# LiWentomng/OrientedRepPoints

Measured on NVIDIA H100. Metric: 1024x1024 tiles/sec, higher is better.
Workload: dtype f16x3

## Files before the change

### orientedreppoints_b200/csrc/common.cuh

```cuda
#pragma once
#include <cuda_runtime.h>
#include <stdint.h>
#include <stdio.h>
#include <string.h>

#include "../../include/orp_b200.h"

namespace orp {

extern thread_local char g_err[512];
extern int64_t g_launches;
extern int g_timing;

inline int fail(int code, const char *fmt, const char *a = "", const char *b = "")
{
    snprintf(g_err, sizeof(g_err), fmt, a, b);
    return code;
}

#define ORP_CUDA(expr)                                                                          \
    do {                                                                                        \
        cudaError_t e__ = (expr);                                                               \
        if (e__ != cudaSuccess) return ::orp::fail(ORP_ECUDA, "%s: %s", #expr, cudaGetErrorString(e__)); \
    } while (0)

#define ORP_LAUNCHED()                                                                          \
    do {                                                                                        \
        __atomic_add_fetch(&::orp::g_launches, 1, __ATOMIC_RELAXED);                            \
        cudaError_t e__ = cudaGetLastError();                                                   \
        if (e__ != cudaSuccess) return ::orp::fail(ORP_ECUDA, "kernel launch: %s", cudaGetErrorString(e__)); \
    } while (0)

inline void count_launches(int n) { __atomic_add_fetch(&g_launches, n, __ATOMIC_RELAXED); }

int ensure_device();

struct Scratch {
    cudaStream_t st;
    void *ptrs[48];
    int n = 0;
    explicit Scratch(cudaStream_t s) : st(s) {}
    ~Scratch() { for (int i = 0; i < n; ++i) cudaFreeAsync(ptrs[i], st); }
    template <typename T> T *get(size_t count)
    {
        void *p = nullptr;
        size_t bytes = (count ? count : 1) * sizeof(T);
        if (n >= 48 || cudaMallocAsync(&p, bytes, st) != cudaSuccess) return nullptr;
        ptrs[n++] = p;
        return static_cast<T *>(p);
    }
};

int run_nms(const float *dets, const int32_t *segments, int n, double thr, int iou_mode, int union_mode,
            int order, int64_t *keep_out, int32_t *num_out, cudaStream_t st, uint8_t *flags_out, bool no_sync,
            int seg_limit ,
            int32_t *overflow_out );

static inline int ceil_div(long long a, long long b) { return (int)((a + b - 1) / b); }

inline int key_bits(uint64_t v)
{
    int b = 1;
    while (b < 64 && (v >> b)) ++b;
    return b;
}

__device__ __forceinline__ uint32_t orderable(float f)
{
    uint32_t u = __float_as_uint(f);
    return (u & 0x80000000u) ? ~u : (u | 0x80000000u);
}

int device_sms(int &sms);

constexpr int kNumSMs = 132;

inline int grid_for(size_t items, int threads)
{
    const size_t g = (items + threads - 1) / threads;
    const size_t cap = kNumSMs * 16;
    return (int)(g < cap ? (g ? g : 1) : cap);
}

}
```

### orientedreppoints_b200/csrc/head_post.cu

```cuda
#include <cub/cub.cuh>

#include "common.cuh"
#include "minrect.cuh"

namespace orp {
namespace {

constexpr int kMaxLevels = 8;
constexpr int kMaxEntries = 80;

struct Levels {
    const float *cls[kMaxEntries], *ref[kMaxEntries];
    int H[kMaxEntries], W[kMaxEntries], stride[kMaxEntries];
    int slot0[kMaxEntries];
    int sort0[kMaxEntries];
    int nent, per_view, B, C, S;
};
static_assert(sizeof(Levels) <= 4000, "the level table is a kernel argument");

__device__ __forceinline__ float sigmoidf_ref(float x) { return 1.0f / (1.0f + expf(-x)); }

__global__ void __launch_bounds__(256)
maxscore_kernel(const __grid_constant__ Levels L, int lev, uint64_t *__restrict__ keys, int32_t *__restrict__ vals)
{
// ... 226 lines not shown
    O.dets = Sc.get<float>(total * 9);
    O.segs = Sc.get<int32_t>(total);
    O.valid = Sc.get<uint8_t>(total);
    O.rp = aug ? nullptr : Sc.get<float>((size_t)B * S * 18);
    O.box = Sc.get<float>((size_t)B * S * 8);
    uint8_t *keep = Sc.get<uint8_t>(total);
    int32_t *counts = Sc.get<int32_t>(B);
    uint64_t *sk1 = Sc.get<uint64_t>(total), *sk2 = Sc.get<uint64_t>(total);
    int32_t *sv1 = Sc.get<int32_t>(total), *sv2 = Sc.get<int32_t>(total);
    size_t tb1 = 0, tb2 = 0;
    if (nsort) cub::DeviceRadixSort::SortPairs(nullptr, tb1, k1, k2, v1, v2, (int)nsort, 0, 64, st);
    const int sel_bits = 32 + key_bits((uint64_t)B - 1);
    cub::DeviceRadixSort::SortPairs(nullptr, tb2, sk1, sk2, sv1, sv2, (int)total, 0, sel_bits, st);
    uint8_t *tmp = Sc.get<uint8_t>(tb1 > tb2 ? tb1 : tb2);
    if (!tmp || !sv2 || !keep) return fail(ORP_ECUDA, "%s: scratch allocation failed", who);

    if (nsort) {
        for (int l = 0; l < L.nent; ++l)
            if (L.sort0[l] >= 0) {
                maxscore_kernel<<<grid_for((size_t)B * H[l] * W[l], 256), 256, 0, st>>>(L, l, k1, v1);
                ORP_LAUNCHED();
            }
        ORP_CUDA(cub::DeviceRadixSort::SortPairs(tmp, tb1, k1, k2, v1, v2, (int)nsort, 0, 64, st));
        count_launches(9);
    }
    const int dgrid = (int)ceil_div((long long)B * S, 128);
    if (aug) decode_kernel<true><<<dgrid, 128, 0, st>>>(L, v2, score_thr, nullptr, view_meta, O);
    else decode_kernel<false><<<dgrid, 128, 0, st>>>(L, v2, score_thr, scale_factor, nullptr, O);
    ORP_LAUNCHED();
    int32_t *nms_ovf = Sc.get<int32_t>(1);
    if (!nms_ovf) return fail(ORP_ECUDA, "%s: scratch allocation failed", who);
    ORP_CUDA(cudaMemsetAsync(nms_ovf, 0, sizeof(int32_t), st));
    rc = run_nms(O.dets, O.segs, (int)total, iou_thr, ORP_NMS_EXACT64, ORP_UNION_NAN_KEEPS, ORP_ORDER_INDEX_ASC, nullptr,
                 nullptr, st, keep, true, B * num_cls, nms_ovf);
    if (rc) return rc;
    ORP_CUDA(cudaMemsetAsync(counts, 0, sizeof(int32_t) * B, st));
    count_kernel<<<dim3(32, B), 256, 0, st>>>(keep, O.valid, (int)per_img, B, counts);
    ORP_LAUNCHED();
    select_keys_kernel<<<grid_for(total, 256), 256, 0, st>>>(keep, O.valid, O.dets, counts, (int)per_img, B, max_per_img, sk1, sv1);
    ORP_LAUNCHED();
    ORP_CUDA(cub::DeviceRadixSort::SortPairs(tmp, tb2, sk1, sk2, sv1, sv2, (int)total, 0, sel_bits, st));
    count_launches((sel_bits + 7) / 8 + 1);
    gather_kernel<<<dim3(ceil_div(max_per_img, 128), B), 128, 0, st>>>(sv2, counts, O.dets, O.rp, O.box, out_scale, (int)per_img,
                                                                     (int)S, num_cls, max_per_img, B, dets_out, labels_out,
                                                                     counts_out, nms_ovf);
    ORP_LAUNCHED();
    return ORP_OK;
}

}
}

extern "C" int orp_head_postprocess(int nlevels, const float *const *cls, const float *const *ref, const int *H,
                                    const int *W, const int *stride, int B, int num_cls, int nms_pre, float score_thr,
                                    double iou_thr, int max_per_img, const float *scale_factor, float *dets_out,
                                    int64_t *labels_out, int32_t *counts_out, void *stream)
{
    return head_post("orp_head_postprocess", 1, nlevels, cls, ref, H, W, stride, B, num_cls, nms_pre, score_thr, iou_thr,
                     max_per_img, scale_factor, nullptr, nullptr, dets_out, labels_out, counts_out, stream);
}

extern "C" int orp_head_postprocess_aug(int nviews, int nlevels, const float *const *cls, const float *const *ref,
                                        const int *H, const int *W, const int *stride, int B, int num_cls, int nms_pre,
                                        float score_thr, double iou_thr, int max_per_img, const float *view_meta,
                                        const float *out_scale, float *dets_out, int64_t *labels_out, int32_t *counts_out,
                                        void *stream)
{
// ... 40 lines not shown
```

### orientedreppoints_b200/csrc/nms.cu

```cuda
#include <cooperative_groups.h>
#include <cub/cub.cuh>
#include <vector>

#include "common.cuh"
#include "geom.cuh"

namespace cg = cooperative_groups;

namespace orp {

struct NmsCounters {
    unsigned long long pairs_swept, pairs_aabb, pairs_clipped, pairs_fp64, edges, suppressing;
    int overflow;
    int rounds;
};

static thread_local int g_last_n;
static thread_local cudaEvent_t g_ev[2] = {nullptr, nullptr};
static thread_local NmsCounters *g_stats_pinned = nullptr;
static thread_local orp_rnms_plan g_last_plan;
static thread_local bool g_have_plan = false;

constexpr float kZeroArea = -2.0f;

__global__ void __launch_bounds__(256)
nms_prep_kernel(const float *__restrict__ dets, int n, uint32_t *__restrict__ score_key, int32_t *__restrict__ iota)
{
    int i = blockIdx.x * blockDim.x + threadIdx.x;
    if (i >= n) return;
    const float *d = dets + (size_t)i * 9;
    const float sc = (__float_as_uint(d[8]) << 1) == 0u ? 0.0f : d[8];
    score_key[i] = ~orderable(sc);
    iota[i] = i;
}

__global__ void __launch_bounds__(256)
nms_rank_kernel(const int32_t *__restrict__ order, int n, int32_t *__restrict__ rank)
{
    int r = blockIdx.x * blockDim.x + threadIdx.x;
    if (r < n) rank[order[r]] = r;
}

struct NmsGlobal {
    unsigned int ymin_key;
    unsigned int maxh_bits;
    unsigned int maxabs_bits;
    double sumh;
    unsigned int count;
};

__device__ __forceinline__ float from_orderable(uint32_t k)
{
    return __uint_as_float((k & 0x80000000u) ? (k & 0x7FFFFFFFu) : ~k);
}

__global__ void __launch_bounds__(256)
nms_boxes_kernel(const float *__restrict__ dets, int n, float4 *__restrict__ baabb, float4 *__restrict__ v01,
                 float4 *__restrict__ v23, float *__restrict__ area, NmsGlobal *__restrict__ G)
{
    __shared__ unsigned int s_ymin, s_maxh, s_cnt, s_maxabs;
    __shared__ float s_sum;
    if (threadIdx.x == 0) { s_ymin = 0xFFFFFFFFu; s_maxh = 0u; s_cnt = 0u; s_sum = 0.f; s_maxabs = 0u; }
    __syncthreads();
    const int i = blockIdx.x * blockDim.x + threadIdx.x;
    if (i < n) {
        const float *d = dets + (size_t)i * 9;
        float c[8];
        bool finite = true;
#pragma unroll
        for (int k = 0; k < 8; ++k) { c[k] = d[k]; finite = finite && isfinite(c[k]); }
        const float xmin = fminf(fminf(c[0], c[2]), fminf(c[4], c[6])), xmax = fmaxf(fmaxf(c[0], c[2]), fmaxf(c[4], c[6]));
        const float ymin = fminf(fminf(c[1], c[3]), fminf(c[5], c[7])), ymax = fmaxf(fmaxf(c[1], c[3]), fmaxf(c[5], c[7]));
        baabb[i] = make_float4(xmin, ymin, xmax, ymax);
        v01[i] = make_float4(c[0], c[1], c[2], c[3]);
        v23[i] = make_float4(c[4], c[5], c[6], c[7]);
        const float ux = c[2] - c[0], uy = c[3] - c[1], vx = c[4] - c[0], vy = c[5] - c[1], wx = c[6] - c[0], wy = c[7] - c[1];
        area[i] = quad_is_convex(c) ? 0.5f * fabsf((ux * vy - uy * vx) + (vx * wy - vy * wx)) : -1.0f;
        if (finite) {
            Pt<double> P[5];
#pragma unroll
            for (int k = 0; k < 4; ++k) { P[k].x = (double)c[2 * k]; P[k].y = (double)c[2 * k + 1]; }
            if (ring_area(P, 4) == 0.0) area[i] = kZeroArea;
        }
        if (finite) {
            atomicMin(&s_ymin, orderable(ymin));
            atomicMax(&s_maxh, __float_as_uint(ymax - ymin));
            atomicMax(&s_maxabs, __float_as_uint(fmaxf(fmaxf(fabsf(xmin), fabsf(xmax)), fmaxf(fabsf(ymin), fabsf(ymax)))));
            atomicAdd(&s_sum, ymax - ymin);
            atomicAdd(&s_cnt, 1u);
        }
    }
    __syncthreads();
    if (threadIdx.x == 0 && s_cnt) {
        atomicMin(&G->ymin_key, s_ymin);
        atomicMax(&G->maxh_bits, s_maxh);
        atomicMax(&G->maxabs_bits, s_maxabs);
        atomicAdd(&G->sumh, (double)s_sum);
        atomicAdd(&G->count, s_cnt);
    }
}

struct Strips {
    float y0, s;
    __device__ __forceinline__ int of(float y) const { return (int)floorf((y - y0) / s); }
};
__device__ __forceinline__ Strips make_strips(const NmsGlobal *G, int R)
{
    Strips S;
    S.y0 = from_orderable(G->ymin_key);
    if (R == 1 || G->count == 0) { S.s = 3.0e38f; return S; }
    const float maxh = __uint_as_float(G->maxh_bits), meanh = (float)(G->sumh / (double)G->count);
    S.s = fmaxf(fmaxf(1.5f * meanh, maxh * (1.0001f / 3.0f)), 1e-6f);
    return S;
}

__global__ void __launch_bounds__(256)
nms_regs_kernel(const float4 *__restrict__ baabb, const int32_t *__restrict__ segments, int n, int R,
                const NmsGlobal *__restrict__ G, uint64_t *__restrict__ keys, int32_t *__restrict__ vals)
{
    const int i = blockIdx.x * blockDim.x + threadIdx.x;
    if (i >= n) return;
    const float4 b = baabb[i];
    const bool finite = isfinite(b.x) && isfinite(b.y) && isfinite(b.z) && isfinite(b.w);
    const Strips S = make_strips(G, R);
    int t0 = 0, t1 = -1;
    if (finite) { t0 = S.of(b.y); t1 = S.of(b.w); if (R == 1) t1 = t0 = 0; if (t1 - t0 > R - 1) t1 = t0 + R - 1; }
    if (R == 1) {
        const uint64_t seg = segments ? (uint64_t)((uint32_t)segments[i] & 0x7FFFFFFFu) : 0ull;
        keys[i] = finite ? ((seg << 32) | orderable(b.x)) : ~0ull;
        vals[i] = i;
        return;
    }
    const uint64_t seg = segments ? (uint64_t)((uint32_t)segments[i] & 0x7FFFu) : 0ull;
    for (int k = 0; k < R; ++k) {
        const int t = t0 + k;
        keys[(size_t)i * R + k] = (t <= t1) ? ((seg << 48) | ((uint64_t)(uint32_t)(t & 0xFFFF) << 32) | orderable(b.x)) : ~0ull;
        vals[(size_t)i * R + k] = i;
    }
}

__global__ void __launch_bounds__(256)
nms_slots_kernel(const uint64_t *__restrict__ keys, const int32_t *__restrict__ vals, const float4 *__restrict__ baabb,
                 const float *__restrict__ area, const int32_t *__restrict__ rank, int m,
                 float4 *__restrict__ aabb_s, int4 *__restrict__ meta_s, int32_t *__restrict__ nvalid)
{
    const int s = blockIdx.x * blockDim.x + threadIdx.x;
    if (s >= m) return;
    const uint64_t k = keys[s];
    const bool valid = (k != ~0ull);
    const int i = vals[s];
    aabb_s[s] = baabb[i];
    meta_s[s] = make_int4((int32_t)(k >> 32), i, __float_as_int(area[i]), rank[i]);
    const bool prev_valid = (s == 0) ? true : (keys[s - 1] != ~0ull);
    if (!valid && prev_valid) *nvalid = s;
    if (valid && s == m - 1) *nvalid = m;
}

__global__ void __launch_bounds__(256)
nms_zero_keys_kernel(const int32_t *__restrict__ order, const int32_t *__restrict__ segments, const float4 *__restrict__ v01,
                     const float4 *__restrict__ v23, const NmsGlobal *__restrict__ G, int n, uint32_t none, float *__restrict__ area,
                     uint32_t *__restrict__ keys)
{
    const int r = blockIdx.x * blockDim.x + threadIdx.x;
    if (r >= n) return;
    const int i = order[r];
    const float4 a = v01[i], b = v23[i];
    Pt<double> P[5];
    P[0].x = a.x; P[0].y = a.y; P[1].x = a.z; P[1].y = a.w; P[2].x = b.x; P[2].y = b.y; P[3].x = b.z; P[3].y = b.w;
    const double S = fmax(1.0, (double)__uint_as_float(G->maxabs_bits));
    const bool deg = fabs(ring_area(P, 4)) <= ldexp(S * S, -36);
    if (deg) area[i] = kZeroArea;
    keys[r] = deg ? (segments ? ((uint32_t)segments[i] & 0x7FFFFFFFu) : 0u) : none;
}

__global__ void __launch_bounds__(256)
nms_zero_list_kernel(const uint32_t *__restrict__ keys, const int32_t *__restrict__ zlist, int n, uint32_t none,
                     int32_t *__restrict__ zpos, int32_t *__restrict__ zhi, int32_t *__restrict__ zbetter)
{
    const int p = blockIdx.x * blockDim.x + threadIdx.x;
    if (p >= n) return;
    const uint32_t k = keys[p];
    if (k == none) return;
    int a = 0, b = p;
    while (a < b) { const int mid = (a + b) >> 1; if (keys[mid] < k) a = mid + 1; else b = mid; }
    int c = p + 1, d = n;
// ... 54 lines not shown
                                           double thr, float *scratch)
{
    if (!both_convex) return -1;
    const float ox = 0.5f * (fmaxf(ba.x, bb.x) + fminf(ba.z, bb.z));
    const float oy = 0.5f * (fmaxf(ba.y, bb.y) + fminf(ba.w, bb.w));
    float a[8], b[8];
#pragma unroll
    for (int k = 0; k < 4; ++k) {
        a[2 * k] = A.c[2 * k] - ox; a[2 * k + 1] = A.c[2 * k + 1] - oy;
        b[2 * k] = B.c[2 * k] - ox; b[2 * k + 1] = B.c[2 * k + 1] - oy;
    }
    FastRes r = fast_quad_pair_s<1>(a, b, scratch);
    const float t = (float)thr;
    const float margin = r.inter * (1.f + t) - t * (r.area_a + r.area_b);
    const float band = 4.f * r.err + 1e-6f * (r.area_a + r.area_b);
    if (fabsf(margin) > band) return margin > 0.f ? 1 : 0;
    return -1;
}

struct SweepParams {
    const float4 *aabb_s;
    const int4 *meta_s;
    const float4 *v01, *v23;
    const int32_t *nvalid;
    const NmsGlobal *G;
    int R;
    int2 *edges;
    int32_t *outdeg;
    int32_t *pending;
    unsigned long long edge_cap;
    NmsCounters *ctr;
    double thr;
    int union_mode;
};

constexpr int kSweepWarps = 8;

__device__ __forceinline__ bool frame_prune(const float *p, const float *q, float kthr_sum)
{
    const float ux = p[2] - p[0], uy = p[3] - p[1];
    const float l2 = ux * ux + uy * uy;
    if (!(l2 > 0.f)) return false;
    float pu0 = 0.f, pu1 = 0.f, pv0 = 0.f, pv1 = 0.f;
    float qu0 = 3.4e38f, qu1 = -3.4e38f, qv0 = 3.4e38f, qv1 = -3.4e38f;
#pragma unroll
    for (int k = 1; k < 4; ++k) {
        const float dx = p[2 * k] - p[0], dy = p[2 * k + 1] - p[1];
        const float a = dx * ux + dy * uy, c = dy * ux - dx * uy;
        pu0 = fminf(pu0, a); pu1 = fmaxf(pu1, a); pv0 = fminf(pv0, c); pv1 = fmaxf(pv1, c);
    }
#pragma unroll
    for (int k = 0; k < 4; ++k) {
        const float dx = q[2 * k] - p[0], dy = q[2 * k + 1] - p[1];
        const float a = dx * ux + dy * uy, c = dy * ux - dx * uy;
        qu0 = fminf(qu0, a); qu1 = fmaxf(qu1, a); qv0 = fminf(qv0, c); qv1 = fmaxf(qv1, c);
    }
    const float ou = fminf(pu1, qu1) - fmaxf(pu0, qu0), ov = fminf(pv1, qv1) - fmaxf(pv0, qv0);
    if (ou <= 0.f || ov <= 0.f) return true;
    return (ou * ov) < 0.998f * kthr_sum * l2;
}

__global__ void __launch_bounds__(kSweepWarps * 32, 4)
nms_sweep_kernel(SweepParams P)
{
    __shared__ int32_t q1[kSweepWarps][64];
    __shared__ int32_t q1r[kSweepWarps][64];
// ... 52 lines not shown
            if (hit) {
                const int at = n1 + __popc(hm & lt);
                q1[wib][at] = mj.y; q1r[wib][at] = mj.w; q1a[wib][at] = __int_as_float(mj.z);
            }
            n1 += __popc(hm);
            __syncwarp();
            while (n1 >= 32 || (!more && n1 > 0)) {
                const int take = n1 < 32 ? n1 : 32;
                bool pass = false;
                int bj = 0, rk_j = 0;
                if (lane < take) {
                    bj = q1[wib][n1 - take + lane];
                    rk_j = q1r[wib][n1 - take + lane];
                    const float area_j = q1a[wib][n1 - take + lane];
                    pass = true;
                    if (area_i >= 0.f && area_j >= 0.f) {
                        float b[8];
                        const float4 t0 = P.v01[bj], t1 = P.v23[bj];
                        b[0] = t0.x; b[1] = t0.y; b[2] = t0.z; b[3] = t0.w; b[4] = t1.x; b[5] = t1.y; b[6] = t1.z; b[7] = t1.w;
                        const float ks = kthr * (area_i + area_j);
                        if (ks > 0.f && (frame_prune(A, b, ks) || frame_prune(b, A, ks))) pass = false;
                    }
                }
                n1 -= take;
                const unsigned pm = __ballot_sync(0xffffffffu, pass);
                if (pm) {
                    unsigned long long basep = 0;
                    if (lane == 0) basep = atomicAdd(&P.ctr->edges, (unsigned long long)__popc(pm));
                    basep = __shfl_sync(0xffffffffu, basep, 0);
                    if (pass) {
                        const unsigned long long pos = basep + __popc(pm & lt);
                        const bool i_worse = rk_i > rk_j;
                        const int lo = i_worse ? bi : bj, hi = i_worse ? bj : bi;
                        if (pos < P.edge_cap) {
                            P.edges[pos] = make_int2(hi, lo);
                            atomicAdd(&P.outdeg[hi], 1);
                            atomicAdd(&P.pending[lo], 1);
                        } else {
                            P.ctr->overflow = 1;
                        }
                    }
                }
                __syncwarp();
            }
            if (!more) break;
        }
    }
#pragma unroll
    for (int o = 16; o > 0; o >>= 1) {
        c_swept += __shfl_down_sync(0xffffffffu, c_swept, o);
        c_aabb += __shfl_down_sync(0xffffffffu, c_aabb, o);
    }
    if (lane == 0) {
        atomicAdd(&P.ctr->pairs_swept, c_swept);
        atomicAdd(&P.ctr->pairs_aabb, c_aabb);
    }
}

__global__ void __launch_bounds__(64)
nms_compat_tiles_kernel(const float4 *__restrict__ v01, const float4 *__restrict__ v23,
                        const int32_t *__restrict__ sg, int n, float thr, int union_mode,
                        int2 *edges, int32_t *indeg, unsigned long long edge_cap, NmsCounters *ctr)
{
    const int nb = (n + 63) / 64;
    long long t = blockIdx.x;
    int rb = 0;
    {
// ... 31 lines not shown
    if (ri >= n) return;
    float p[8];
    {
        float4 a = v01[ri], b = v23[ri];
        p[0] = a.x; p[1] = a.y; p[2] = a.z; p[3] = a.w; p[4] = b.x; p[5] = b.y; p[6] = b.z; p[7] = b.w;
    }
    const int seg_i = sg[ri];
    const int ncol = min(64, n - cb * 64);
    const int start = (rb == cb) ? threadIdx.x + 1 : 0;
    unsigned long long clipped = 0;
    for (int c = start; c < ncol; ++c) {
        if (colseg[c] != seg_i) continue;
        float q[8];
#pragma unroll
        for (int k = 0; k < 8; ++k) q[k] = col[c][k];
        PairRes<float> r = ref_quad_pair<float>(p, q);
        float iou = iou_from<float>(r, union_mode);
        ++clipped;
        if (suppresses<float>(iou, thr, union_mode)) {
            unsigned long long pos = atomicAdd(&ctr->edges, 1ull);
            if (pos < edge_cap) {
                const int lo = cb * 64 + c, hi = ri;
                edges[pos] = make_int2(lo, hi);
                atomicAdd(&indeg[lo], 1);
            } else {
                ctr->overflow = 1;
            }
        }
    }
    atomicAdd(&ctr->pairs_clipped, clipped);
}

__global__ void __launch_bounds__(256)
nms_scatter_kernel(const int2 *__restrict__ edges, const NmsCounters *__restrict__ ctr,
                   unsigned long long edge_cap, const int32_t *__restrict__ offs,
                   int32_t *__restrict__ cursor, int32_t *__restrict__ adj)
{
    unsigned long long ne = ctr->edges < edge_cap ? ctr->edges : edge_cap;
    for (unsigned long long e = blockIdx.x * (unsigned long long)blockDim.x + threadIdx.x; e < ne;
         e += (unsigned long long)gridDim.x * blockDim.x) {
        int2 ed = edges[e];
        int pos = offs[ed.x] + atomicAdd(&cursor[ed.x], 1);
        adj[pos] = ed.y;
    }
}

__global__ void __launch_bounds__(256)
nms_resolve_kernel(const int32_t *__restrict__ offs, const int32_t *__restrict__ adj, int n,
                   volatile uint8_t *status, int *changed , NmsCounters *ctr)
{
    cg::grid_group grid = cg::this_grid();
    const int tid = blockIdx.x * blockDim.x + threadIdx.x;
    const int nth = gridDim.x * blockDim.x;
    int round = 0;
    while (true) {
        int *flag = &changed[round & 1];
        int local = 0;
        for (int r = tid; r < n; r += nth) {
            if (status[r] != 0) continue;
            const int b = offs[r], e = offs[r + 1];
            bool any_keep = false, all_supp = true;
            for (int k = b; k < e; ++k) {
                const uint8_t s = status[adj[k]];
                if (s == 1) { any_keep = true; break; }
                if (s == 0) all_supp = false;
            }
            if (any_keep) { status[r] = 2; local = 1; }
            else if (all_supp) { status[r] = 1; local = 1; }
        }
        if (local) *flag = 1;
        __threadfence();
        grid.sync();
        const int any = *(volatile int *)flag;
        if (tid == 0) changed[(round + 1) & 1] = 0;
        ++round;
        grid.sync();
        if (!any) break;
    }
    if (tid == 0) ctr->rounds = round;
}

struct LazyParams {
    const int32_t *offs;
    const int32_t *adj;
    const int32_t *deg;
    int n;
    int32_t *status;
    int32_t *pending;
    NmsCounters *ctr;
    unsigned int *counts;
    int32_t *fkept, *fsup;
    int2 *queue;
    const float4 *aabb, *v01, *v23;
    const float *area;
    double thr;
    int union_mode;
    const int32_t *zlist, *zpos, *zhi;
};

__global__ void __launch_bounds__(256, 4)
nms_resolve_lazy_kernel(LazyParams P)
{
    cg::grid_group grid = cg::this_grid();
    float scratch[40];
    const int tid = blockIdx.x * blockDim.x + threadIdx.x;
    const int nth = gridDim.x * blockDim.x;
    const int lane = threadIdx.x & 31, gwarp = tid >> 5, nwarps = nth >> 5;
    const unsigned lt = (1u << lane) - 1u;
    unsigned long long c_clip = 0, c_64 = 0, c_sup = 0;
    for (int r0 = blockIdx.x * blockDim.x; r0 < P.n; r0 += nth) {
        const int r = r0 + threadIdx.x;
        const bool k = r < P.n && P.pending[r] == 0;
        const unsigned m = __ballot_sync(0xffffffffu, k);
        if (m) {
            unsigned int base = 0;
            if (lane == 0) base = atomicAdd(&P.counts[0], (unsigned int)__popc(m));
            base = __shfl_sync(0xffffffffu, base, 0);
            if (k) { P.status[r] = 1; P.fkept[base + __popc(m & lt)] = r; }
        }
    }
    __threadfence();
    grid.sync();
    int round = 0;
    while (true) {
        const int cur = round & 1, nxt = cur ^ 1;
        const unsigned int nk = *(volatile unsigned int *)&P.counts[cur];
        const unsigned int ns = *(volatile unsigned int *)&P.counts[2 + cur];
        if (nk == 0 && ns == 0) break;
        const int32_t *fk = P.fkept + (size_t)cur * P.n, *fs = P.fsup + (size_t)cur * P.n;
        int32_t *fk_next = P.fkept + (size_t)nxt * P.n, *fs_next = P.fsup + (size_t)nxt * P.n;
// ... 23 lines not shown
                            if (m) {
                                unsigned int base = 0;
                                if (lane == 0) base = atomicAdd(qc, (unsigned int)__popc(m));
                                base = __shfl_sync(0xffffffffu, base, 0);
                                if (act[u]) P.queue[base + __popc(m & lt)] = make_int2(r[u], j);
                            }
                        }
                    } else {
    #pragma unroll
                        for (int u = 0; u < 4; ++u)
                            if (act[u] && atomicSub(&P.pending[r[u]], 1) == 1) {
                                P.status[r[u]] = 1;
                                fk_next[atomicAdd(&P.counts[nxt], 1u)] = r[u];
                            }
                    }
                }
            }
        }
        __threadfence();
        grid.sync();
        const unsigned int nq = *(volatile unsigned int *)qc;
        if (tid == 0) { P.counts[cur] = 0; P.counts[2 + cur] = 0; P.counts[4 + nxt] = 0; }
        for (unsigned int q0 = (unsigned int)(tid - lane); q0 < nq; q0 += nth) {
            const unsigned int q = q0 + lane;
            int r = -1, j = -1, res = 0;
            bool valid = q < nq;
            Quad A, B;
            if (valid) {
                const int2 e = P.queue[q];
                r = e.x; j = e.y;
                valid = *(volatile int32_t *)&P.status[r] == 0;
            }
            if (valid) {
                const float4 t0 = P.v01[r], t1 = P.v23[r];
                A.c[0] = t0.x; A.c[1] = t0.y; A.c[2] = t0.z; A.c[3] = t0.w; A.c[4] = t1.x; A.c[5] = t1.y; A.c[6] = t1.z; A.c[7] = t1.w;
                const float4 u0 = P.v01[j], u1 = P.v23[j];
                B.c[0] = u0.x; B.c[1] = u0.y; B.c[2] = u0.z; B.c[3] = u0.w; B.c[4] = u1.x; B.c[5] = u1.y; B.c[6] = u1.z; B.c[7] = u1.w;
                res = decide_fast(A, B, P.aabb[r], P.aabb[j], P.area[r] >= 0.f && P.area[j] >= 0.f, P.thr, scratch);
                ++c_clip;
            }
            unsigned hard = __ballot_sync(0xffffffffu, valid && res < 0);
            while (hard) {
                const int src = __ffs(hard) - 1;
                hard &= hard - 1;
                Quad HA, HB;
#pragma unroll
                for (int k = 0; k < 8; ++k) {
                    HA.c[k] = __shfl_sync(0xffffffffu, A.c[k], src);
                    HB.c[k] = __shfl_sync(0xffffffffu, B.c[k], src);
                }
                const bool s = decide_fp64_warp(HB, HA, P.thr, P.union_mode, lane);
                if (lane == src) { res = s ? 1 : 0; ++c_64; }
            }
            if (!valid) continue;
            if (res) {
                ++c_sup;
                if (atomicExch(&P.status[r], 2) == 0) fs_next[atomicAdd(&P.counts[2 + nxt], 1u)] = r;
            } else if (atomicSub(&P.pending[r], 1) == 1) {
                P.status[r] = 1;
                fk_next[atomicAdd(&P.counts[nxt], 1u)] = r;
            }
        }
        ++round;
        __threadfence();
        grid.sync();
    }
#pragma unroll
    for (int o = 16; o > 0; o >>= 1) {
        c_clip += __shfl_down_sync(0xffffffffu, c_clip, o);
        c_64 += __shfl_down_sync(0xffffffffu, c_64, o);
        c_sup += __shfl_down_sync(0xffffffffu, c_sup, o);
// ... 13 lines not shown

__global__ void __launch_bounds__(256)
nms_flags_kernel(const uint8_t *__restrict__ status, const int32_t *__restrict__ status_orig, const int32_t *__restrict__ order,
                 const int32_t *__restrict__ rank, int n, int out_order,
                 uint8_t *__restrict__ flags, int64_t *__restrict__ vals)
{
    int k = blockIdx.x * blockDim.x + threadIdx.x;
    if (k >= n) return;
    if (out_order == ORP_ORDER_SCORE_DESC) {
        flags[k] = (status_orig ? status_orig[order[k]] : (int32_t)status[k]) == 1;
        vals[k] = order[k];
    } else {
        flags[k] = (status_orig ? status_orig[k] : (int32_t)status[rank[k]]) == 1;
        vals[k] = k;
    }
}

static int launch_resolve(const void *kernel, int need, void **args, cudaStream_t st)
{
    int sms = 0, per_sm = 0;
    const int rc = device_sms(sms);
    if (rc) return rc;
    ORP_CUDA(cudaOccupancyMaxActiveBlocksPerMultiprocessor(&per_sm, kernel, 256, 0));
    if (per_sm > 4) per_sm = 4;
    int grid = sms * (per_sm > 0 ? per_sm : 1);
    if (grid > need) grid = need;
    ORP_CUDA(cudaLaunchCooperativeKernel(kernel, dim3(grid), dim3(256), args, 0, st));
    ORP_LAUNCHED();
    return ORP_OK;
}

int run_nms(const float *dets, const int32_t *segments, int n, double thr, int iou_mode, int union_mode,
            int order, int64_t *keep_out, int32_t *num_out, cudaStream_t st, uint8_t *flags_out, bool no_sync, int seg_limit,
            int32_t *overflow_out)
{
    if (!segments) seg_limit = 1;
    if (n < 0 || (!flags_out && !num_out) || (n > 0 && (!dets || (!flags_out && !keep_out))))
        return fail(ORP_EINVAL, "orp_rnms: null pointer or negative n");
    if (iou_mode != ORP_NMS_EXACT64 && iou_mode != ORP_NMS_COMPAT32) return fail(ORP_EINVAL, "orp_rnms: bad iou_mode");
    if (union_mode < 0 || union_mode > 3) return fail(ORP_EINVAL, "orp_rnms: bad union_mode");
    int rc = ensure_device();
    if (rc) return rc;
    const bool lazy = (iou_mode == ORP_NMS_EXACT64);
    memset(&g_last_plan, 0, sizeof(g_last_plan));
    g_last_plan.lazy = lazy; g_last_plan.seg_limit = seg_limit; g_last_plan.no_sync = no_sync; g_last_plan.flags_out = flags_out != nullptr;
    g_last_plan.union_mode = union_mode; g_last_plan.order = order; g_last_plan.n = n;
    g_have_plan = true;
    if (n == 0) {
        if (num_out) ORP_CUDA(cudaMemsetAsync(num_out, 0, sizeof(int32_t), st));
        return ORP_OK;
    }
    const bool zero_rule = lazy && (union_mode == ORP_UNION_GUARD || union_mode == ORP_UNION_NAN_SUPPRESSES_ALL);
    const long long per_seg = seg_limit > 0 ? (long long)n / seg_limit : (long long)n;
    const int R = (lazy && per_seg >= 16384 && seg_limit > 0 && seg_limit <= 32767) ? 4 : 1;
    const int m = n * R;
    const int sweep_bits = seg_limit > 0 ? (R == 1 ? 32 : 48) + key_bits((uint64_t)seg_limit) : 64;
    const int zbits = seg_limit > 0 ? key_bits((uint64_t)seg_limit) : 32;
    const uint32_t znone = zbits == 32 ? 0xFFFFFFFFu : (uint32_t)((1ull << zbits) - 1);
    unsigned long long cap = (unsigned long long)n * 256ull;
    if (cap < (1ull << 20)) cap = 1ull << 20;
    const unsigned long long all_pairs = (unsigned long long)n * (unsigned long long)(n - 1) / 2ull;
    if (cap > all_pairs) cap = all_pairs ? all_pairs : 1;
    g_last_plan.R = R; g_last_plan.sweep_bits = sweep_bits;
    g_last_plan.cap_first = g_last_plan.cap_final = (int64_t)cap;
    Scratch S(st);
    const int T = 256, G = ceil_div(n, T), GM = ceil_div(m, T);
    uint32_t *score_key = S.get<uint32_t>(n), *score_key2 = S.get<uint32_t>(n);
    int32_t *iota = S.get<int32_t>(m), *order_r = S.get<int32_t>(n), *rank = S.get<int32_t>(n);
    float4 *v01 = S.get<float4>(n), *v23 = S.get<float4>(n);
    int32_t *list_len = S.get<int32_t>(n + 1), *offs = S.get<int32_t>(n + 1), *cursor = S.get<int32_t>(n + 1);
    uint8_t *flags = flags_out ? flags_out : S.get<uint8_t>(n);
    int64_t *vals = S.get<int64_t>(n);
    NmsCounters *ctr = S.get<NmsCounters>(1);
    uint64_t *sweep_key = lazy ? S.get<uint64_t>(m) : nullptr, *sweep_key2 = lazy ? S.get<uint64_t>(m) : nullptr;
    int32_t *perm = lazy ? S.get<int32_t>(m) : nullptr, *nvalid = lazy ? S.get<int32_t>(1) : nullptr;
    float4 *baabb = lazy ? S.get<float4>(n) : nullptr, *aabb_s = lazy ? S.get<float4>(m) : nullptr;
    int4 *meta_s = lazy ? S.get<int4>(m) : nullptr;
    float *area = lazy ? S.get<float>(n) : nullptr;
    NmsGlobal *glob = lazy ? S.get<NmsGlobal>(1) : nullptr;
    unsigned int *qcount = lazy ? S.get<unsigned int>(6) : nullptr;
    int32_t *worklist = lazy ? S.get<int32_t>(4 * (size_t)n) : nullptr;
    int32_t *status32 = lazy ? S.get<int32_t>(n) : nullptr, *pending = lazy ? S.get<int32_t>(n) : nullptr;
    int32_t *zlist = zero_rule ? S.get<int32_t>(n) : nullptr, *zpos = zero_rule ? S.get<int32_t>(n) : nullptr;
    int32_t *zhi = zero_rule ? S.get<int32_t>(n) : nullptr, *zbetter = zero_rule ? S.get<int32_t>(n) : nullptr;
    int32_t *sg = lazy ? nullptr : S.get<int32_t>(n);
    uint8_t *status = lazy ? nullptr : S.get<uint8_t>(n);
    int *changed = lazy ? nullptr : S.get<int>(2);
    if (!ctr || !vals || !flags || (lazy && (!worklist || !status32 || !pending || !meta_s || !qcount || !glob)) ||
        (zero_rule && (!zlist || !zpos || !zhi || !zbetter)) || (!lazy && (!sg || !status || !changed)))
        return fail(ORP_ECUDA, "orp_rnms: scratch allocation failed");

    size_t tb1 = 0, tb2 = 0, tb3 = 0, tb4 = 0, tb5 = 0;
    cub::DeviceRadixSort::SortPairs(nullptr, tb1, score_key, score_key2, iota, order_r, n, 0, 32, st);
    if (lazy) cub::DeviceRadixSort::SortPairs(nullptr, tb2, sweep_key, sweep_key2, iota, perm, m, 0, sweep_bits, st);
    if (zero_rule) cub::DeviceRadixSort::SortPairs(nullptr, tb5, score_key, score_key2, order_r, zlist, n, 0, zbits, st);
    cub::DeviceScan::ExclusiveSum(nullptr, tb3, list_len, offs, n + 1, st);
    if (keep_out && num_out) cub::DeviceSelect::Flagged(nullptr, tb4, vals, flags, keep_out, num_out, n, st);
    size_t tb = tb1 > tb2 ? tb1 : tb2;
    tb = tb > tb3 ? tb : tb3;
    tb = tb > tb4 ? tb : tb4;
    tb = tb > tb5 ? tb : tb5;
    uint8_t *tmp = S.get<uint8_t>(tb);
    if (!tmp) return fail(ORP_ECUDA, "orp_rnms: scratch allocation failed");

    ORP_CUDA(cudaMemsetAsync(ctr, 0, sizeof(NmsCounters), st));
    ORP_CUDA(cudaMemsetAsync(list_len, 0, sizeof(int32_t) * (size_t)(n + 1), st));
    ORP_CUDA(cudaMemsetAsync(cursor, 0, sizeof(int32_t) * (size_t)(n + 1), st));

    nms_prep_kernel<<<G, T, 0, st>>>(dets, n, score_key, iota);
    ORP_LAUNCHED();
    ORP_CUDA(cub::DeviceRadixSort::SortPairs(tmp, tb1, score_key, score_key2, iota, order_r, n, 0, 32, st));
    count_launches(4);
    nms_rank_kernel<<<G, T, 0, st>>>(order_r, n, rank);
    ORP_LAUNCHED();

    if (lazy) {
        ORP_CUDA(cudaMemsetAsync(pending, 0, sizeof(int32_t) * (size_t)n, st));
        ORP_CUDA(cudaMemsetAsync(glob, 0, sizeof(NmsGlobal), st));
        ORP_CUDA(cudaMemsetAsync(&glob->ymin_key, 0xFF, sizeof(glob->ymin_key), st));
        nms_boxes_kernel<<<G, T, 0, st>>>(dets, n, baabb, v01, v23, area, glob);
        ORP_LAUNCHED();
        nms_regs_kernel<<<G, T, 0, st>>>(baabb, segments, n, R, glob, sweep_key, iota);
        ORP_LAUNCHED();
        ORP_CUDA(cub::DeviceRadixSort::SortPairs(tmp, tb2, sweep_key, sweep_key2, iota, perm, m, 0, sweep_bits, st));
        count_launches((sweep_bits + 7) / 8);
        nms_slots_kernel<<<GM, T, 0, st>>>(sweep_key2, perm, baabb, area, rank, m, aabb_s, meta_s, nvalid);
        ORP_LAUNCHED();
        if (zero_rule) {
            ORP_CUDA(cudaMemsetAsync(zpos, 0xFF, sizeof(int32_t) * (size_t)n, st));
            nms_zero_keys_kernel<<<G, T, 0, st>>>(order_r, segments, v01, v23, glob, n, znone, area, score_key);
            ORP_LAUNCHED();
            ORP_CUDA(cub::DeviceRadixSort::SortPairs(tmp, tb5, score_key, score_key2, order_r, zlist, n, 0, zbits, st));
            count_launches((zbits + 7) / 8);
            nms_zero_list_kernel<<<G, T, 0, st>>>(score_key2, zlist, n, znone, zpos, zhi, zbetter);
            ORP_LAUNCHED();
        }
    } else {
        nms_gather_kernel<<<G, T, 0, st>>>(dets, segments, order_r, n, v01, v23, sg);
        ORP_LAUNCHED();
    }

    int2 *edges = nullptr;
    for (int attempt = 0; attempt < 6; ++attempt) {
        g_last_plan.attempts = attempt + 1;
        g_last_plan.cap_final = (int64_t)cap;
        edges = S.get<int2>(cap + (zero_rule ? (unsigned long long)n : 0ull));
        if (!edges) return fail(ORP_ECUDA, "orp_rnms: edge buffer allocation failed");
        if (lazy) {
            SweepParams P{aabb_s, meta_s, v01, v23, nvalid, glob, R, edges, list_len, pending, cap, ctr, thr, union_mode};
            int grid = ceil_div(m, kSweepWarps);
            const int maxgrid = kNumSMs * 8 * 4;
            if (grid > maxgrid) grid = maxgrid;
            if (g_timing) {
                if (!g_ev[0]) { ORP_CUDA(cudaEventCreate(&g_ev[0])); ORP_CUDA(cudaEventCreate(&g_ev[1])); }
                ORP_CUDA(cudaEventRecord(g_ev[0], st));
            }
            nms_sweep_kernel<<<grid, kSweepWarps * 32, 0, st>>>(P);
            ORP_LAUNCHED();
            if (g_timing) ORP_CUDA(cudaEventRecord(g_ev[1], st));
        } else {
            const long long nb = (n + 63) / 64;
            const long long tiles = nb * (nb + 1) / 2;
            if (tiles > 2147483647LL) return fail(ORP_EINVAL, "orp_rnms: n too large for COMPAT32 mode");
            nms_compat_tiles_kernel<<<(unsigned)tiles, 64, 0, st>>>(v01, v23, sg, n, (float)thr, union_mode, edges,
                                                                    list_len, cap, ctr);
            ORP_LAUNCHED();
        }
        if (cap >= all_pairs || no_sync) break;
        NmsCounters h;
        ORP_CUDA(cudaMemcpyAsync(&h, ctr, sizeof(h), cudaMemcpyDeviceToHost, st));
        ORP_CUDA(cudaStreamSynchronize(st));
        if (!h.overflow) break;
        if (attempt == 5) return fail(ORP_EOVERFLOW, "orp_rnms: edge buffer overflow");
        cap = h.edges + h.edges / 8 + 1024;
        if (cap > all_pairs) cap = all_pairs;
        ORP_CUDA(cudaMemsetAsync(ctr, 0, sizeof(NmsCounters), st));
        ORP_CUDA(cudaMemsetAsync(list_len, 0, sizeof(int32_t) * (size_t)(n + 1), st));
        if (lazy) ORP_CUDA(cudaMemsetAsync(pending, 0, sizeof(int32_t) * (size_t)n, st));
    }
    if (zero_rule) {
        nms_zero_pending_kernel<<<G, T, 0, st>>>(zpos, zbetter, n, pending);
        ORP_LAUNCHED();
    }

    ORP_CUDA(cub::DeviceScan::ExclusiveSum(tmp, tb3, list_len, offs, n + 1, st));
    count_launches(2);
    int32_t *adj = S.get<int32_t>(cap);
    if (!adj) return fail(ORP_ECUDA, "orp_rnms: adjacency allocation failed");
    nms_scatter_kernel<<<kNumSMs * 8, 256, 0, st>>>(edges, ctr, cap, offs, cursor, adj);
    ORP_LAUNCHED();
    if (lazy) {
        ORP_CUDA(cudaMemsetAsync(status32, 0, sizeof(int32_t) * (size_t)n, st));
        ORP_CUDA(cudaMemsetAsync(qcount, 0, 6 * sizeof(unsigned int), st));
        LazyParams LP{offs, adj, cursor, n, status32, pending, ctr, qcount, worklist, worklist + 2 * (size_t)n, edges,
                      baabb, v01, v23, area, thr, union_mode, zlist, zpos, zhi};
        void *args[] = {&LP};
        rc = launch_resolve((const void *)nms_resolve_lazy_kernel, ceil_div(n, 8), args, st);
    } else {
        ORP_CUDA(cudaMemsetAsync(status, 0, (size_t)n, st));
        ORP_CUDA(cudaMemsetAsync(changed, 0, 2 * sizeof(int), st));
        void *args[] = {&offs, &adj, &n, &status, &changed, &ctr};
        rc = launch_resolve((const void *)nms_resolve_kernel, ceil_div(n, 256), args, st);
    }
    if (rc) return rc;
    if (overflow_out) {
        nms_export_overflow_kernel<<<1, 1, 0, st>>>(ctr, overflow_out);
        ORP_LAUNCHED();
    }
    nms_flags_kernel<<<G, T, 0, st>>>(status, status32, order_r, rank, n, flags_out ? ORP_ORDER_INDEX_ASC : order, flags, vals);
    ORP_LAUNCHED();
    if (keep_out && num_out) {
        if (flags_out && order != ORP_ORDER_INDEX_ASC) return fail(ORP_EINVAL, "orp_rnms: flags_out needs index order");
        ORP_CUDA(cub::DeviceSelect::Flagged(tmp, tb4, vals, flags, keep_out, num_out, n, st));
        count_launches(3);
    }

    if (!g_stats_pinned) ORP_CUDA(cudaHostAlloc(&g_stats_pinned, sizeof(NmsCounters), cudaHostAllocDefault));
    ORP_CUDA(cudaMemcpyAsync(g_stats_pinned, ctr, sizeof(NmsCounters), cudaMemcpyDeviceToHost, st));
    g_last_n = n;
    return ORP_OK;
}

}

extern "C" int orp_rnms(const float *dets, const int32_t *segments, int n, double iou_thr, int iou_mode,
                        int union_mode, int order, int64_t *keep_out, int32_t *num_out, void *stream)
{
    return orp::run_nms(dets, segments, n, iou_thr, iou_mode, union_mode, order, keep_out, num_out,
// ... 76 lines not shown
```

Baseline: 322.9.

## Share box geometry across classes in rotated NMS sweep

When every class of a location shares one decoded box, the NMS now builds AABBs, sorts and sweeps only the unique boxes, then expands each overlapping box pair into per-class edges in a new expand kernel. The resolve step indexes geometry by box rather than by detection. This cuts the sort and sweep work by the number of classes, at the cost of an extra pair buffer and an expansion pass. A fixed pair capacity with no host-side retry adds a risk of overflow.

```diff
diff --git a/orientedreppoints_b200/csrc/common.cuh b/orientedreppoints_b200/csrc/common.cuh
--- a/orientedreppoints_b200/csrc/common.cuh
+++ b/orientedreppoints_b200/csrc/common.cuh
@@ -54,7 +54,8 @@
 int run_nms(const float *dets, const int32_t *segments, int n, double thr, int iou_mode, int union_mode,
             int order, int64_t *keep_out, int32_t *num_out, cudaStream_t st, uint8_t *flags_out, bool no_sync,
             int seg_limit ,
-            int32_t *overflow_out );
+            int32_t *overflow_out ,
+            const float *boxes = nullptr, int share = 1);
 
 static inline int ceil_div(long long a, long long b) { return (int)((a + b - 1) / b); }
 
diff --git a/orientedreppoints_b200/csrc/head_post.cu b/orientedreppoints_b200/csrc/head_post.cu
--- a/orientedreppoints_b200/csrc/head_post.cu
+++ b/orientedreppoints_b200/csrc/head_post.cu
@@ -282,7 +282,7 @@
     if (!nms_ovf) return fail(ORP_ECUDA, "%s: scratch allocation failed", who);
     ORP_CUDA(cudaMemsetAsync(nms_ovf, 0, sizeof(int32_t), st));
     rc = run_nms(O.dets, O.segs, (int)total, iou_thr, ORP_NMS_EXACT64, ORP_UNION_NAN_KEEPS, ORP_ORDER_INDEX_ASC, nullptr,
-                 nullptr, st, keep, true, B * num_cls, nms_ovf);
+                 nullptr, st, keep, true, B * num_cls, nms_ovf, O.box, num_cls);
     if (rc) return rc;
     ORP_CUDA(cudaMemsetAsync(counts, 0, sizeof(int32_t) * B, st));
     count_kernel<<<dim3(32, B), 256, 0, st>>>(keep, O.valid, (int)per_img, B, counts);
diff --git a/orientedreppoints_b200/csrc/nms.cu b/orientedreppoints_b200/csrc/nms.cu
--- a/orientedreppoints_b200/csrc/nms.cu
+++ b/orientedreppoints_b200/csrc/nms.cu
@@ -55,7 +55,7 @@
 }
 
 __global__ void __launch_bounds__(256)
-nms_boxes_kernel(const float *__restrict__ dets, int n, float4 *__restrict__ baabb, float4 *__restrict__ v01,
+nms_boxes_kernel(const float *__restrict__ dets, int n, int stride, float4 *__restrict__ baabb, float4 *__restrict__ v01,
                  float4 *__restrict__ v23, float *__restrict__ area, NmsGlobal *__restrict__ G)
 {
     __shared__ unsigned int s_ymin, s_maxh, s_cnt, s_maxabs;
@@ -64,7 +64,7 @@
     __syncthreads();
     const int i = blockIdx.x * blockDim.x + threadIdx.x;
     if (i < n) {
-        const float *d = dets + (size_t)i * 9;
+        const float *d = dets + (size_t)i * stride;
         float c[8];
         bool finite = true;
 #pragma unroll
@@ -115,23 +115,24 @@
 }
 
 __global__ void __launch_bounds__(256)
-nms_regs_kernel(const float4 *__restrict__ baabb, const int32_t *__restrict__ segments, int n, int R,
+nms_regs_kernel(const float4 *__restrict__ baabb, const int32_t *__restrict__ segments, int share, int n, int R,
                 const NmsGlobal *__restrict__ G, uint64_t *__restrict__ keys, int32_t *__restrict__ vals)
 {
     const int i = blockIdx.x * blockDim.x + threadIdx.x;
     if (i >= n) return;
+    const int32_t sid = segments ? segments[(size_t)i * share] / share : 0;
     const float4 b = baabb[i];
     const bool finite = isfinite(b.x) && isfinite(b.y) && isfinite(b.z) && isfinite(b.w);
     const Strips S = make_strips(G, R);
     int t0 = 0, t1 = -1;
     if (finite) { t0 = S.of(b.y); t1 = S.of(b.w); if (R == 1) t1 = t0 = 0; if (t1 - t0 > R - 1) t1 = t0 + R - 1; }
     if (R == 1) {
-        const uint64_t seg = segments ? (uint64_t)((uint32_t)segments[i] & 0x7FFFFFFFu) : 0ull;
+        const uint64_t seg = (uint64_t)((uint32_t)sid & 0x7FFFFFFFu);
         keys[i] = finite ? ((seg << 32) | orderable(b.x)) : ~0ull;
         vals[i] = i;
         return;
     }
-    const uint64_t seg = segments ? (uint64_t)((uint32_t)segments[i] & 0x7FFFu) : 0ull;
+    const uint64_t seg = (uint64_t)((uint32_t)sid & 0x7FFFu);
     for (int k = 0; k < R; ++k) {
         const int t = t0 + k;
         keys[(size_t)i * R + k] = (t <= t1) ? ((seg << 48) | ((uint64_t)(uint32_t)(t & 0xFFFF) << 32) | orderable(b.x)) : ~0ull;
@@ -150,7 +151,7 @@
     const bool valid = (k != ~0ull);
     const int i = vals[s];
     aabb_s[s] = baabb[i];
-    meta_s[s] = make_int4((int32_t)(k >> 32), i, __float_as_int(area[i]), rank[i]);
+    meta_s[s] = make_int4((int32_t)(k >> 32), i, __float_as_int(area[i]), rank ? rank[i] : 0);
     const bool prev_valid = (s == 0) ? true : (keys[s - 1] != ~0ull);
     if (!valid && prev_valid) *nvalid = s;
     if (valid && s == m - 1) *nvalid = m;
@@ -271,6 +272,7 @@
     NmsCounters *ctr;
     double thr;
     int union_mode;
+    bool pairs_only;
 };
 
 constexpr int kSweepWarps = 8;
@@ -389,7 +391,9 @@
                         const unsigned long long pos = basep + __popc(pm & lt);
                         const bool i_worse = rk_i > rk_j;
                         const int lo = i_worse ? bi : bj, hi = i_worse ? bj : bi;
-                        if (pos < P.edge_cap) {
+                        if (pos < P.edge_cap && P.pairs_only) {
+                            P.edges[pos] = make_int2(bi, bj);
+                        } else if (pos < P.edge_cap) {
                             P.edges[pos] = make_int2(hi, lo);
                             atomicAdd(&P.outdeg[hi], 1);
                             atomicAdd(&P.pending[lo], 1);
@@ -487,6 +491,56 @@
 }
 
 __global__ void __launch_bounds__(256)
+nms_expand_kernel(const int2 *__restrict__ pairs, const NmsCounters *__restrict__ pctr, unsigned long long pair_cap,
+                  const float *__restrict__ dets, const int32_t *__restrict__ rank, int share, int2 *__restrict__ edges,
+                  int32_t *__restrict__ outdeg, int32_t *__restrict__ pending, unsigned long long edge_cap,
+                  NmsCounters *__restrict__ ctr)
+{
+    const int lane = threadIdx.x & 31;
+    const unsigned lt = (1u << lane) - 1u;
+    if (blockIdx.x == 0 && threadIdx.x == 0) {
+        ctr->pairs_swept = pctr->pairs_swept;
+        ctr->pairs_aabb = pctr->pairs_aabb;
+        if (pctr->overflow) ctr->overflow = 1;
+    }
+    const unsigned long long np = pctr->edges < pair_cap ? pctr->edges : pair_cap;
+    const unsigned long long total = np * (unsigned long long)share;
+    for (unsigned long long w0 = blockIdx.x * (unsigned long long)blockDim.x + (threadIdx.x & ~31u); w0 < total;
+         w0 += (unsigned long long)gridDim.x * blockDim.x) {
+        const unsigned long long t = w0 + lane;
+        bool pass = false;
+        int hi = 0, lo = 0;
+        if (t < total) {
+            const int2 p = pairs[t / share];
+            const int c = (int)(t % share);
+            const int ra = p.x * share + c, rb = p.y * share + c;
+            const float *da = dets + (size_t)ra * 9, *db = dets + (size_t)rb * 9;
+            pass = true;
+#pragma unroll
+            for (int k = 0; k < 8; ++k) pass = pass && isfinite(da[k]) && isfinite(db[k]);
+            const bool a_worse = rank[ra] > rank[rb];
+            hi = a_worse ? rb : ra;
+            lo = a_worse ? ra : rb;
+        }
+        const unsigned pm = __ballot_sync(0xffffffffu, pass);
+        if (!pm) continue;
+        unsigned long long base = 0;
+        if (lane == 0) base = atomicAdd(&ctr->edges, (unsigned long long)__popc(pm));
+        base = __shfl_sync(0xffffffffu, base, 0);
+        if (pass) {
+            const unsigned long long pos = base + __popc(pm & lt);
+            if (pos < edge_cap) {
+                edges[pos] = make_int2(hi, lo);
+                atomicAdd(&outdeg[hi], 1);
+                atomicAdd(&pending[lo], 1);
+            } else {
+                ctr->overflow = 1;
+            }
+        }
+    }
+}
+
+__global__ void __launch_bounds__(256)
 nms_scatter_kernel(const int2 *__restrict__ edges, const NmsCounters *__restrict__ ctr,
                    unsigned long long edge_cap, const int32_t *__restrict__ offs,
                    int32_t *__restrict__ cursor, int32_t *__restrict__ adj)
@@ -551,6 +605,7 @@
     double thr;
     int union_mode;
     const int32_t *zlist, *zpos, *zhi;
+    int share;
 };
 
 __global__ void __launch_bounds__(256, 4)
@@ -640,11 +695,12 @@
                 valid = *(volatile int32_t *)&P.status[r] == 0;
             }
             if (valid) {
-                const float4 t0 = P.v01[r], t1 = P.v23[r];
+                const int gr = r / P.share, gj = j / P.share;
+                const float4 t0 = P.v01[gr], t1 = P.v23[gr];
                 A.c[0] = t0.x; A.c[1] = t0.y; A.c[2] = t0.z; A.c[3] = t0.w; A.c[4] = t1.x; A.c[5] = t1.y; A.c[6] = t1.z; A.c[7] = t1.w;
-                const float4 u0 = P.v01[j], u1 = P.v23[j];
+                const float4 u0 = P.v01[gj], u1 = P.v23[gj];
                 B.c[0] = u0.x; B.c[1] = u0.y; B.c[2] = u0.z; B.c[3] = u0.w; B.c[4] = u1.x; B.c[5] = u1.y; B.c[6] = u1.z; B.c[7] = u1.w;
-                res = decide_fast(A, B, P.aabb[r], P.aabb[j], P.area[r] >= 0.f && P.area[j] >= 0.f, P.thr, scratch);
+                res = decide_fast(A, B, P.aabb[gr], P.aabb[gj], P.area[gr] >= 0.f && P.area[gj] >= 0.f, P.thr, scratch);
                 ++c_clip;
             }
             unsigned hard = __ballot_sync(0xffffffffu, valid && res < 0);
@@ -724,13 +780,17 @@
 
 int run_nms(const float *dets, const int32_t *segments, int n, double thr, int iou_mode, int union_mode,
             int order, int64_t *keep_out, int32_t *num_out, cudaStream_t st, uint8_t *flags_out, bool no_sync, int seg_limit,
-            int32_t *overflow_out)
+            int32_t *overflow_out, const float *boxes, int share)
 {
     if (!segments) seg_limit = 1;
     if (n < 0 || (!flags_out && !num_out) || (n > 0 && (!dets || (!flags_out && !keep_out))))
         return fail(ORP_EINVAL, "orp_rnms: null pointer or negative n");
     if (iou_mode != ORP_NMS_EXACT64 && iou_mode != ORP_NMS_COMPAT32) return fail(ORP_EINVAL, "orp_rnms: bad iou_mode");
     if (union_mode < 0 || union_mode > 3) return fail(ORP_EINVAL, "orp_rnms: bad union_mode");
+    if (!boxes) share = 1;
+    if (boxes && (share < 1 || n % share || !segments || iou_mode != ORP_NMS_EXACT64 || union_mode != ORP_UNION_NAN_KEEPS ||
+                  !no_sync))
+        return fail(ORP_EINVAL, "orp_rnms: shared boxes need segments, EXACT64, ORP_UNION_NAN_KEEPS and no host sync");
     int rc = ensure_device();
     if (rc) return rc;
     const bool lazy = (iou_mode == ORP_NMS_EXACT64);
@@ -745,7 +805,8 @@
     const bool zero_rule = lazy && (union_mode == ORP_UNION_GUARD || union_mode == ORP_UNION_NAN_SUPPRESSES_ALL);
     const long long per_seg = seg_limit > 0 ? (long long)n / seg_limit : (long long)n;
     const int R = (lazy && per_seg >= 16384 && seg_limit > 0 && seg_limit <= 32767) ? 4 : 1;
-    const int m = n * R;
+    const int nbox = n / share;
+    const int m = nbox * R;
     const int sweep_bits = seg_limit > 0 ? (R == 1 ? 32 : 48) + key_bits((uint64_t)seg_limit) : 64;
     const int zbits = seg_limit > 0 ? key_bits((uint64_t)seg_limit) : 32;
     const uint32_t znone = zbits == 32 ? 0xFFFFFFFFu : (uint32_t)((1ull << zbits) - 1);
@@ -758,17 +819,17 @@
     Scratch S(st);
     const int T = 256, G = ceil_div(n, T), GM = ceil_div(m, T);
     uint32_t *score_key = S.get<uint32_t>(n), *score_key2 = S.get<uint32_t>(n);
-    int32_t *iota = S.get<int32_t>(m), *order_r = S.get<int32_t>(n), *rank = S.get<int32_t>(n);
-    float4 *v01 = S.get<float4>(n), *v23 = S.get<float4>(n);
+    int32_t *iota = S.get<int32_t>(m > n ? m : n), *order_r = S.get<int32_t>(n), *rank = S.get<int32_t>(n);
+    float4 *v01 = S.get<float4>(nbox), *v23 = S.get<float4>(nbox);
     int32_t *list_len = S.get<int32_t>(n + 1), *offs = S.get<int32_t>(n + 1), *cursor = S.get<int32_t>(n + 1);
     uint8_t *flags = flags_out ? flags_out : S.get<uint8_t>(n);
     int64_t *vals = S.get<int64_t>(n);
     NmsCounters *ctr = S.get<NmsCounters>(1);
     uint64_t *sweep_key = lazy ? S.get<uint64_t>(m) : nullptr, *sweep_key2 = lazy ? S.get<uint64_t>(m) : nullptr;
     int32_t *perm = lazy ? S.get<int32_t>(m) : nullptr, *nvalid = lazy ? S.get<int32_t>(1) : nullptr;
-    float4 *baabb = lazy ? S.get<float4>(n) : nullptr, *aabb_s = lazy ? S.get<float4>(m) : nullptr;
+    float4 *baabb = lazy ? S.get<float4>(nbox) : nullptr, *aabb_s = lazy ? S.get<float4>(m) : nullptr;
     int4 *meta_s = lazy ? S.get<int4>(m) : nullptr;
-    float *area = lazy ? S.get<float>(n) : nullptr;
+    float *area = lazy ? S.get<float>(nbox) : nullptr;
     NmsGlobal *glob = lazy ? S.get<NmsGlobal>(1) : nullptr;
     unsigned int *qcount = lazy ? S.get<unsigned int>(6) : nullptr;
     int32_t *worklist = lazy ? S.get<int32_t>(4 * (size_t)n) : nullptr;
@@ -810,13 +871,15 @@
         ORP_CUDA(cudaMemsetAsync(pending, 0, sizeof(int32_t) * (size_t)n, st));
         ORP_CUDA(cudaMemsetAsync(glob, 0, sizeof(NmsGlobal), st));
         ORP_CUDA(cudaMemsetAsync(&glob->ymin_key, 0xFF, sizeof(glob->ymin_key), st));
-        nms_boxes_kernel<<<G, T, 0, st>>>(dets, n, baabb, v01, v23, area, glob);
+        const int GB = ceil_div(nbox, T);
+        if (boxes) nms_boxes_kernel<<<GB, T, 0, st>>>(boxes, nbox, 8, baabb, v01, v23, area, glob);
+        else nms_boxes_kernel<<<GB, T, 0, st>>>(dets, nbox, 9, baabb, v01, v23, area, glob);
         ORP_LAUNCHED();
-        nms_regs_kernel<<<G, T, 0, st>>>(baabb, segments, n, R, glob, sweep_key, iota);
+        nms_regs_kernel<<<GB, T, 0, st>>>(baabb, segments, share, nbox, R, glob, sweep_key, iota);
         ORP_LAUNCHED();
         ORP_CUDA(cub::DeviceRadixSort::SortPairs(tmp, tb2, sweep_key, sweep_key2, iota, perm, m, 0, sweep_bits, st));
         count_launches((sweep_bits + 7) / 8);
-        nms_slots_kernel<<<GM, T, 0, st>>>(sweep_key2, perm, baabb, area, rank, m, aabb_s, meta_s, nvalid);
+        nms_slots_kernel<<<GM, T, 0, st>>>(sweep_key2, perm, baabb, area, boxes ? nullptr : rank, m, aabb_s, meta_s, nvalid);
         ORP_LAUNCHED();
         if (zero_rule) {
             ORP_CUDA(cudaMemsetAsync(zpos, 0xFF, sizeof(int32_t) * (size_t)n, st));
@@ -832,6 +895,19 @@
         ORP_LAUNCHED();
     }
 
+    unsigned long long pair_cap = 0;
+    int2 *pairs = nullptr;
+    NmsCounters *pctr = nullptr;
+    if (boxes) {
+        pair_cap = (unsigned long long)nbox * 256ull;
+        if (pair_cap < (1ull << 20)) pair_cap = 1ull << 20;
+        const unsigned long long box_pairs = (unsigned long long)nbox * (unsigned long long)(nbox - 1) / 2ull;
+        if (pair_cap > box_pairs) pair_cap = box_pairs ? box_pairs : 1;
+        pairs = S.get<int2>(pair_cap);
+        pctr = S.get<NmsCounters>(1);
+        if (!pairs || !pctr) return fail(ORP_ECUDA, "orp_rnms: scratch allocation failed");
+        ORP_CUDA(cudaMemsetAsync(pctr, 0, sizeof(NmsCounters), st));
+    }
     int2 *edges = nullptr;
     for (int attempt = 0; attempt < 6; ++attempt) {
         g_last_plan.attempts = attempt + 1;
@@ -839,7 +915,8 @@
         edges = S.get<int2>(cap + (zero_rule ? (unsigned long long)n : 0ull));
         if (!edges) return fail(ORP_ECUDA, "orp_rnms: edge buffer allocation failed");
         if (lazy) {
-            SweepParams P{aabb_s, meta_s, v01, v23, nvalid, glob, R, edges, list_len, pending, cap, ctr, thr, union_mode};
+            SweepParams P{aabb_s, meta_s, v01, v23, nvalid, glob, R, boxes ? pairs : edges, list_len, pending,
+                          boxes ? pair_cap : cap, boxes ? pctr : ctr, thr, union_mode, boxes != nullptr};
             int grid = ceil_div(m, kSweepWarps);
             const int maxgrid = kNumSMs * 8 * 4;
             if (grid > maxgrid) grid = maxgrid;
@@ -850,6 +927,11 @@
             nms_sweep_kernel<<<grid, kSweepWarps * 32, 0, st>>>(P);
             ORP_LAUNCHED();
             if (g_timing) ORP_CUDA(cudaEventRecord(g_ev[1], st));
+            if (boxes) {
+                nms_expand_kernel<<<kNumSMs * 8, 256, 0, st>>>(pairs, pctr, pair_cap, dets, rank, share, edges, list_len, pending,
+                                                               cap, ctr);
+                ORP_LAUNCHED();
+            }
         } else {
             const long long nb = (n + 63) / 64;
             const long long tiles = nb * (nb + 1) / 2;
@@ -885,7 +967,7 @@
         ORP_CUDA(cudaMemsetAsync(status32, 0, sizeof(int32_t) * (size_t)n, st));
         ORP_CUDA(cudaMemsetAsync(qcount, 0, 6 * sizeof(unsigned int), st));
         LazyParams LP{offs, adj, cursor, n, status32, pending, ctr, qcount, worklist, worklist + 2 * (size_t)n, edges,
-                      baabb, v01, v23, area, thr, union_mode, zlist, zpos, zhi};
+                      baabb, v01, v23, area, thr, union_mode, zlist, zpos, zhi, share};
         void *args[] = {&LP};
         rc = launch_resolve((const void *)nms_resolve_lazy_kernel, ceil_div(n, 8), args, st);
     } else {
```

Result: no change. 325.9 (median of 6 runs) (+0.9%).
